# lschoe/mpyc

Hardware: AMD Instinct MI355X
Metric: field-ops/sec (modmul + share+recombine) on 10^7-elt SecFld array (higher is better)
Workload: dtype u64; 1 GPU; configs[1]: SecFld(GF(2^61-1)) array, 10^7 elements per GPU; step = modmul + np_random_split(m=3,t=1, coefficients supplied) + np_recombine(k=3); modmul is fused into the share-generation kernel (product never written to HBM); n_per_gpu=10000000, prime=2^61-1, m=3, t=1, k=3, buffer_sets=4, parallelism=element-sharded x1, no collective

## Files before the change

### mpyc_amd/csrc/api.hip

```cpp
#include <hip/hip_runtime.h>
#include <stdint.h>
#include <stdio.h>
#include <stdlib.h>
#include <string.h>
#include <limits.h>
#include <mutex>
#include <new>

#include "../../include/ffgpu.h"
#include "../../include/ffgpu_math.h"
#include "handoff.hpp"
#include "kernels.hpp"
#include "policy_build.hpp"

using namespace ffgpu;

const FieldOps* ffgpu_ops_pm64_mersenne();
const FieldOps* ffgpu_ops_pm64_k64();
const FieldOps* ffgpu_ops_pm64_gen();
const FieldOps* ffgpu_ops_rc64();
const FieldOps* ffgpu_ops_rc32();
const FieldOps* ffgpu_ops_pm128_k128();
const FieldOps* ffgpu_ops_pm128_gen();
const FieldOps* ffgpu_ops_pm96();
// ... 137 lines not shown

static void acc_harvest(ffgpu_ctx* c) {
    if (c->acc_n == 0) return;
    (void)hipEventSynchronize(c->acc_ev[2 * (c->acc_n - 1) + 1]);
    for (int i = 0; i < c->acc_n; ++i) {
        float ms = 0.f;
        if (hipEventElapsedTime(&ms, c->acc_ev[2 * i], c->acc_ev[2 * i + 1]) == hipSuccess) c->acc_ms += ms;
    }
    c->acc_calls += (unsigned long long)c->acc_n;
    c->acc_n = 0;
}

struct LaunchTimer {
    ffgpu_ctx* c;
    hipStream_t st;
    int slot;
    LaunchTimer(ffgpu_ctx* ctx, hipStream_t s) : c(ctx && ctx->timing ? ctx : nullptr), st(s), slot(-1) {
        if (!c) return;
        if (c->timing == 2) {
            if (c->acc_n == ffgpu_ctx::ACC_MAX) acc_harvest(c);
            if (c->acc_n == c->acc_made) {
                if (hipEventCreate(&c->acc_ev[2 * c->acc_made]) != hipSuccess ||
                    hipEventCreate(&c->acc_ev[2 * c->acc_made + 1]) != hipSuccess) {
                    c = nullptr;
                    return;
                }
                ++c->acc_made;
            }
            slot = c->acc_n++;
            (void)hipEventRecord(c->acc_ev[2 * slot], st);
        } else {
            (void)hipEventRecord(c->ev0, st);
        }
    }
    ~LaunchTimer() {
        if (!c) return;
        if (slot >= 0) {
            (void)hipEventRecord(c->acc_ev[2 * slot + 1], st);
        } else {
            (void)hipEventRecord(c->ev1, st);
            c->timed = 1;
        }
    }
};

struct CallScope {
    DeviceGuard dev;
    LaunchTimer timer;
    hipStream_t st;
    LaunchCfg lc;
    CallScope(ffgpu_ctx* ctx, void* stream)
        : dev(ctx->device), timer(ctx, (hipStream_t)stream), st((hipStream_t)stream), lc(ctx->lc) {}
    CallScope(ffgpu_ctx* ctx, void* stream, int kind, const ByteRange* in, int nin, const ByteRange& out) : CallScope(ctx, stream) {
        if (lc.handoff) {
            std::lock_guard<std::mutex> lk(ctx->handoff_mu);
            int fed = 0;
            const int keep = ctx->handoff.launch(stream, kind, in, nin, &out, 1, &fed);
            lc.policy = (keep ? (kind == HK_SPLIT ? CP_ST_SC1 : CP_ST_PLAIN) : CP_ST_NT) | (fed ? CP_FED : 0);
        }
    }
};

static const FieldOps* ops_for(int kind) {
    switch (kind) {
        case POL_PM64_MERSENNE: return ffgpu_ops_pm64_mersenne();
        case POL_PM64_K64: return ffgpu_ops_pm64_k64();
        case POL_PM64_GEN: return ffgpu_ops_pm64_gen();
        case POL_RC64: return ffgpu_ops_rc64();
        case POL_RC32: return ffgpu_ops_rc32();
        case POL_PM128_K128: return ffgpu_ops_pm128_k128();
        case POL_PM128_GEN: return ffgpu_ops_pm128_gen();
        case POL_PM96: return ffgpu_ops_pm96();
        case POL_PM192: return ffgpu_ops_pm192();
        case POL_MONT192: return ffgpu_ops_mont192();
        case POL_MONT128: return ffgpu_ops_mont128();
        case POL_GF2P8: return ffgpu_ops_gf2p8();
        case POL_GF2W32: return ffgpu_ops_gf2w32();
        case POL_GF2W64: return ffgpu_ops_gf2w64();
        case POL_GF2W128: return ffgpu_ops_gf2w128();
        default: return nullptr;
    }
}

extern "C" {

int ffgpu_abi_version(void) { return FFGPU_ABI_VERSION; }

const char* ffgpu_strerror(int status) {
    switch (status) {
        case FFGPU_OK: return "ok";
        case FFGPU_EINVAL: return "invalid argument";
        case FFGPU_ENOTSUP: return "field or size not supported by this build";
        case FFGPU_EHIP: return "HIP runtime error";
        case FFGPU_ESTALE: return "interprocess mapping does not show the exported row (stale mapping)";
        case FFGPU_EMODULUS: return "unusable modulus";
        case FFGPU_ENOMEM: return "out of device memory";
        default: return "unknown status";
    }
}

const char* ffgpu_last_hip_error(void) { return g_hip_err; }

int ffgpu_device_count(int* count) {
    if (!count) return FFGPU_EINVAL;
    int n = 0;
    hipError_t e = hipGetDeviceCount(&n);
    if (e != hipSuccess) {
        *count = 0;
        return hip_fail(e, "hipGetDeviceCount");
    }
    *count = n;
    return FFGPU_OK;
}

int ffgpu_device_pci_bus_id(int device, char* buf, int len) {
    if (!buf || len < 16 || device < 0) return FFGPU_EINVAL;
    buf[0] = 0;
    hipError_t e = hipDeviceGetPCIBusId(buf, len, device);
    if (e != hipSuccess) return hip_fail(e, "hipDeviceGetPCIBusId");
    return FFGPU_OK;
}

struct Switch {
    const char* name;
    int LaunchCfg::*field;
    double LaunchCfg::*real;
    double def;
    int lowest, highest;
};
static const Switch SWITCHES[] = {
    {"FFGPU_BLOCKS_PER_CU", &LaunchCfg::blocks_per_cu, nullptr, 0, 0, INT_MAX},
    {"FFGPU_MM_MFMA", &LaunchCfg::mm_mfma, nullptr, 1, INT_MIN, INT_MAX},
    {"FFGPU_MM_MFMA_MIN", nullptr, &LaunchCfg::mm_mfma_min, 8e7, 0, 0},
    {"FFGPU_MM_STACK_LOOP_MIN", &LaunchCfg::mm_stack_loop_min, nullptr, 1 << 22, 0, INT_MAX},
    {"FFGPU_GF2W_BITSLICED", &LaunchCfg::gf2w_bitsliced, nullptr, 1, INT_MIN, INT_MAX},
    {"FFGPU_HANDOFF", &LaunchCfg::handoff, nullptr, 1, INT_MIN, INT_MAX},
    {"FFGPU_CONV_WIDE_PER_CU", &LaunchCfg::conv_wide_per_cu, nullptr, 2, 0, INT_MAX},
    {"FFGPU_SCAN_GEOM", &LaunchCfg::scan_geom, nullptr, 0, 0, 2},
    {"FFGPU_SCAN_TILE_THREADS", &LaunchCfg::scan_tile_threads, nullptr, 256, 1, 256},
};

int ffgpu_ctx_create(int kind, const uint64_t* modulus, int nlimbs, int device, ffgpu_ctx** out) {
    if (!modulus || !out || nlimbs < 1 || nlimbs > 3 || device < 0) return FFGPU_EINVAL;
    PolicyBlob pb;
    memset(&pb, 0, sizeof(pb));
    int rc;
    if (kind == FFGPU_PRIME) {
        rc = build_prime_policy3(&pb, modulus, nlimbs);
    } else if (kind == FFGPU_BINARY) {
        rc = build_binary_policy(&pb, modulus, nlimbs);
    } else {
        rc = FFGPU_EINVAL;
    }
    if (rc != FFGPU_OK) return rc;
    if (!ops_for(pb.kind)) return FFGPU_ENOTSUP;
    ffgpu_ctx* c = new (std::nothrow) ffgpu_ctx();
    if (!c) return FFGPU_ENOMEM;
    c->ops = ops_for(pb.kind);
    c->kind = kind;
    c->device = device;
    for (int i = 0; i < nlimbs; ++i) c->modulus[i] = modulus[i];
    memcpy(c->policy, pb.bytes, sizeof(c->policy));
    c->reduction = pb.reduction;
    c->elem_bytes = pb.elem_bytes;
    c->policy_kind = pb.kind;
    rng_const(pb, c->rng_r);
    {
        int cus = 256;
        if (hipDeviceGetAttribute(&cus, hipDeviceAttributeMultiprocessorCount, device) != hipSuccess || cus <= 0) cus = 256;
        c->lc.num_cu = cus;
        for (const Switch& sw : SWITCHES) {
            const char* e = getenv(sw.name);
            if (sw.real) {
                c->lc.*sw.real = e ? atof(e) : sw.def;
                continue;
            }
            const int v = e ? atoi(e) : (int)sw.def;
            c->lc.*sw.field = v >= sw.lowest && v <= sw.highest ? v : (int)sw.def;
        }
    }
    if (pb.kind == POL_GF2W64 || pb.kind == POL_GF2W128) {
        bool in_regs;
        if (pb.kind == POL_GF2W128) {
            GF2W128 f;
            memcpy(&f, pb.bytes, sizeof(f));
            in_regs = (f.fast & 1) != 0;
        } else {
            GF2W64 f;
            memcpy(&f, pb.bytes, sizeof(f));
// ... 430 lines not shown
                void* dev_singular, void* stream) {
    ARGCHK(ctx && n >= 0 && ncols >= n && (mode == 0 || mode == 1));
    if (batch == 0) return FFGPU_OK;
    ARGCHK(dev_singular && (mode == 0 || det_out));
    if (n == 0) return FFGPU_OK;
    ARGCHK(a);
    CallScope cs(ctx, stream);
    ExpArgs ex;
    inverse_exponent(ctx, &ex);
    HIPCHK(hipMemsetAsync(dev_singular, 0, batch * sizeof(int), cs.st));
    return status_of(ctx->ops->gauss(ctx->policy, cs.lc, a, n, ncols, batch, mode, &ex,
                                     mode ? det_out : nullptr, (int*)dev_singular, cs.st));
}

int ffgpu_inv(ffgpu_ctx* ctx, const void* a, void* out, size_t n, void* dev_zero_flag, void* stream) {
    ARGCHK(ctx);
    if (n == 0) return FFGPU_OK;
    ARGCHK(a && out);
    ExpArgs ex;
    inverse_exponent(ctx, &ex);
    CallScope cs(ctx, stream);
    return status_of(ctx->ops->inv(ctx->policy, cs.lc, a, &ex, out, n, (int*)dev_zero_flag, cs.st));
}

int ffgpu_beaver_combine(ffgpu_ctx* ctx, const void* z, const void* x, const void* y, const void* d, const void* e,
                         int add_de, void* out, size_t n, void* stream) {
    ARGCHK(ctx);
    if (n == 0) return FFGPU_OK;
    ARGCHK(z && x && y && d && e && out);
    CallScope cs(ctx, stream);
    return status_of(ctx->ops->beaver(ctx->policy, cs.lc, z, x, y, d, e, out, add_de ? 1 : 0, n,
                                      cs.st));
}

static int split_inputs(const ffgpu_ctx* ctx, const void* a, const void* b, const void* coeffs, int t, size_t coeff_stride, size_t n,
                        ByteRange in[3]) {
    int nin = 0;
    in[nin++] = byte_range(a, rows_bytes(ctx, 1, 0, n));
    if (b) in[nin++] = byte_range(b, rows_bytes(ctx, 1, 0, n));
    if (coeffs) in[nin++] = byte_range(coeffs, rows_bytes(ctx, (size_t)t, coeff_stride, n));
    return nin;
}

static int do_split(ffgpu_ctx* ctx, const void* a, const void* b, bool fused, const void* coeffs,
                    size_t coeff_stride, int t, int m, void* shares, size_t share_stride, size_t n,
                    void* stream) {
    ARGCHK(ctx);
    ARGCHK(m >= 1 && t >= 0 && t < m);
    if (n == 0) return FFGPU_OK;
    ARGCHK(a && shares && (!fused || b) && (t == 0 || coeffs));
    ARGCHK((m == 1 || share_stride >= n) && (t <= 1 || coeff_stride >= n));
    ByteRange in[3];
    const int nin = split_inputs(ctx, a, fused ? b : nullptr, t > 0 ? coeffs : nullptr, t, coeff_stride, n, in);
    CallScope cs(ctx, stream, HK_SPLIT, in, nin, byte_range(shares, rows_bytes(ctx, (size_t)m, share_stride, n)));
    return status_of(ctx->ops->split(ctx->policy, cs.lc, a, fused ? b : nullptr, coeffs,
                                     coeff_stride, t, m, shares, share_stride, n, cs.st,
                                     nullptr));
}

static int make_rng(const ffgpu_ctx* ctx, const uint8_t* key32, uint64_t nonce, int rounds, RngArgs* ra) {
    if (!key32) return FFGPU_EINVAL;
    if (rounds == 0) rounds = 20;
    if (rounds != 20 && rounds != 12 && rounds != 8) return FFGPU_EINVAL;
    memset(ra, 0, sizeof(*ra));
    memcpy(ra->rk.key, key32, 32);
    ra->rk.nonce[0] = (uint32_t)nonce;
    ra->rk.nonce[1] = (uint32_t)(nonce >> 32);
    ra->rk.rounds = (uint32_t)rounds;
    ra->r0 = ctx->rng_r[0];
    ra->r1 = ctx->rng_r[1];
    return FFGPU_OK;
}

static RngArgs make_dev_rng(const ffgpu_ctx* ctx, void* dev_state, uint64_t nonce_off, int defer_advance, bool sampler) {
    RngArgs ra;
    memset(&ra, 0, sizeof(ra));
    ra.rk.rounds = 20;
    if (sampler) {
        ra.r0 = ctx->rng_r[0];
        ra.r1 = ctx->rng_r[1];
    }
    ra.dev_key = (const RngKey*)dev_state;
    ra.nonce_off = (uint32_t)nonce_off;
    ra.no_advance = defer_advance ? 1 : 0;
    return ra;
}

static int do_split_rng(ffgpu_ctx* ctx, const void* a, const void* b, bool fused, const uint8_t* key32,
                        uint64_t nonce, int rounds, int t, int m, void* shares, size_t share_stride, size_t n,
                        void* stream) {
    ARGCHK(ctx);
    ARGCHK(m >= 1 && t >= 0 && t < m);
    RngArgs ra;
    int rc = make_rng(ctx, key32, nonce, rounds, &ra);
    if (rc != FFGPU_OK) return rc;
    if (n == 0) return FFGPU_OK;
    ARGCHK(a && shares && (!fused || b));
    ARGCHK(m == 1 || share_stride >= n);
    ByteRange in[3];
    const int nin = split_inputs(ctx, a, fused ? b : nullptr, nullptr, 0, 0, n, in);
    CallScope cs(ctx, stream, HK_SPLIT, in, nin, byte_range(shares, rows_bytes(ctx, (size_t)m, share_stride, n)));
    if (fused && t > 0) ra.aux = gf8_tables_on_device(ctx);
    return status_of(ctx->ops->split(ctx->policy, cs.lc, a, fused ? b : nullptr, nullptr, 0, t, m,
                                     shares, share_stride, n, cs.st, t > 0 ? &ra : nullptr));
}
int ffgpu_ctx_scalar_limbs(const ffgpu_ctx* ctx) { return (ctx && ctx->elem_bytes == 24) ? 3 : 2; }

size_t ffgpu_rng_state_bytes(void) { return sizeof(RngKey); }

int ffgpu_rng_state_init(ffgpu_ctx* ctx, void* dev_state, const uint8_t* host_key32, uint64_t nonce, int rounds,
                         void* stream) {
    ARGCHK(ctx && dev_state);
    RngArgs ra;
    int rc = make_rng(ctx, host_key32, nonce, rounds, &ra);
    if (rc != FFGPU_OK) return rc;
    CallScope cs(ctx, stream);
    HIPCHK(hipMemcpyAsync(dev_state, &ra.rk, sizeof(RngKey), hipMemcpyHostToDevice, cs.st));
    HIPCHK(hipStreamSynchronize(cs.st));
    return FFGPU_OK;
}

int ffgpu_split_rng_state(ffgpu_ctx* ctx, const void* secrets, const void* mul_by, void* dev_state, int t, int m,
                          void* shares, size_t share_stride, size_t n, void* stream) {
    ARGCHK(ctx && dev_state);
    ARGCHK(m >= 1 && t >= 0 && t < m);
    if (n == 0) return FFGPU_OK;
    ARGCHK(secrets && shares && (m == 1 || share_stride >= n));
    RngArgs ra = make_dev_rng(ctx, dev_state, 0, 0, true);
    ByteRange in[3];
    const int nin = split_inputs(ctx, secrets, mul_by, nullptr, 0, 0, n, in);
    CallScope cs(ctx, stream, HK_SPLIT, in, nin, byte_range(shares, rows_bytes(ctx, (size_t)m, share_stride, n)));
    if (mul_by && t > 0) ra.aux = gf8_tables_on_device(ctx);
    return status_of(ctx->ops->split(ctx->policy, cs.lc, secrets, mul_by, nullptr, 0, t, m, shares, share_stride, n, cs.st,
                                     t > 0 ? &ra : nullptr));
}

int ffgpu_gate_rng(ffgpu_ctx* ctx, const void* const* host_rows_a, const uint64_t* host_lambda_a, int ka,
                   const void* const* host_rows_b, const uint64_t* host_lambda_b, int kb, const uint8_t* host_key32,
                   uint64_t nonce, int rounds, void* dev_state, int t, int m, void* shares, size_t share_stride,
                   size_t n, void* stream) {
    return ffgpu_gate_rng_batch(ctx, host_rows_a, host_lambda_a, ka, 0, host_rows_b, host_lambda_b, kb, 0, host_key32,
                                dev_state ? 0 : nonce, rounds, dev_state, 0, t, m, shares, share_stride, 0, n, 1, stream);
}

int ffgpu_rng_state_advance(ffgpu_ctx* ctx, void* dev_state, uint32_t by, void* stream) {
    ARGCHK(ctx && dev_state);
    if (by == 0) return FFGPU_OK;
    DeviceGuard g(ctx->device);
    hipLaunchKernelGGL((k_rng_advance<0>), dim3(1), dim3(1), 0, (hipStream_t)stream, (RngKey*)dev_state, by);
    return status_of(launched());
}

int ffgpu_gate_rng_batch(ffgpu_ctx* ctx, const void* const* host_rows_a, const uint64_t* host_lambda_a, int ka,
                         size_t batch_stride_a, const void* const* host_rows_b, const uint64_t* host_lambda_b, int kb,
                         size_t batch_stride_b, const uint8_t* host_key32, uint64_t nonce, int rounds, void* dev_state,
                         int defer_advance, int t, int m, void* shares, size_t share_stride, size_t batch_stride_out,
                         size_t n, int nbatch, void* stream) {
    ARGCHK(ctx);
    ARGCHK(nbatch >= 1 && nbatch <= 255);
    ARGCHK(!dev_state || nonce <= 0xffffffffull);
    ARGCHK(dev_state || nbatch == 1 || nonce < (1ull << 40));
    ARGCHK(m >= 1 && t >= 1 && t < m && ka >= 1 && kb >= 0);
    if (t > 3 || ka > 7 || kb > 7) return FFGPU_ENOTSUP;
    ARGCHK(host_rows_a && host_lambda_a && (kb == 0 || (host_rows_b && host_lambda_b)));
    RngArgs ra;
    if (dev_state) {
        ra = make_dev_rng(ctx, dev_state, nonce, defer_advance, true);
    } else {
        int rc = make_rng(ctx, host_key32, nonce, rounds, &ra);
        if (rc != FFGPU_OK) return rc;
    }
    if (n == 0) return FFGPU_OK;
    ARGCHK(shares && (m == 1 || share_stride >= n));
    for (int j = 0; j < ka; ++j) ARGCHK(host_rows_a[j]);
    for (int j = 0; j < kb; ++j) ARGCHK(host_rows_b[j]);
    ByteRange in[14];
    int nin = 0;
    for (int j = 0; j < ka; ++j) in[nin++] = byte_range(host_rows_a[j], rows_bytes(ctx, (size_t)nbatch, batch_stride_a, n));
    for (int j = 0; j < kb; ++j) in[nin++] = byte_range(host_rows_b[j], rows_bytes(ctx, (size_t)nbatch, batch_stride_b, n));
    const size_t oelems = ((size_t)nbatch - 1) * batch_stride_out + ((size_t)m - 1) * share_stride + n;
    CallScope cs(ctx, stream, HK_SPLIT, in, nin, byte_range(shares, oelems * (size_t)ctx->elem_bytes));
    ra.aux = gf8_tables_on_device(ctx);
    return status_of(ctx->ops->gate(ctx->policy, cs.lc, host_rows_a, host_lambda_a, ka, host_rows_b,
                                    host_lambda_b, kb, t, m, shares, share_stride, n, cs.st, &ra,
// ... 1112 lines not shown
```

### mpyc_amd/csrc/handoff.hpp

```cpp
#pragma once
#include <stddef.h>
#include <stdint.h>

namespace ffgpu {

struct ByteRange {
    uintptr_t lo, hi;
};
inline ByteRange byte_range(const void* p, size_t bytes) {
    const uintptr_t lo = (uintptr_t)p;
    return {lo, lo + bytes};
}
inline bool overlaps(const ByteRange& a, const ByteRange& b) { return a.lo < b.hi && b.lo < a.hi && a.lo < a.hi && b.lo < b.hi; }

enum HandoffKind { HK_EW = 0, HK_SPLIT = 1, HK_REC = 2, HK_COPY = 3, HK_KINDS = 4 };

struct HandoffTracker {
    enum { STREAMS = 8, ROWS = 8 };
    static constexpr size_t MAX_KEEP_BYTES = (size_t)256 << 20;
    struct Lane {
        const void* stream;
        uint64_t stamp;
        int used;
        int kind;
        int nout;
        int kept;
        ByteRange out[ROWS];
        uint8_t keep[HK_KINDS];
    } lanes[STREAMS];
    uint64_t clock;

    void reset() {
        for (Lane& l : lanes) {
            l.stream = nullptr;
            l.stamp = 0;
            l.used = 0;
            l.kind = 0;
            l.nout = 0;
            l.kept = 0;
            for (uint8_t& k : l.keep) k = 0;
        }
        clock = 0;
    }
    Lane& lane_of(const void* stream) {
        Lane* victim = nullptr;
        for (Lane& l : lanes) {
            if (l.used && l.stream == stream) return l;
            if (!victim || (!l.used && victim->used) || (l.used == victim->used && l.stamp < victim->stamp)) victim = &l;
        }
        Lane& l = *victim;
        l.stream = stream;
        l.used = 1;
        l.nout = 0;
        l.kept = 0;
        for (uint8_t& k : l.keep) k = 0;
        return l;
    }
    int launch(const void* stream, int kind, const ByteRange* in, int nin, const ByteRange* out, int nout, int* fed_in = nullptr) {
        Lane& l = lane_of(stream);
        l.stamp = ++clock;
        bool fed = false;
        if (l.nout > 0) {
            for (int i = 0; i < nin && !fed; ++i)
                for (int j = 0; j < l.nout && !fed; ++j) fed = overlaps(in[i], l.out[j]);
            l.keep[l.kind] = fed ? 1 : 0;
        }
        if (fed_in) *fed_in = fed && l.kept;
        size_t bytes = 0;
        for (int j = 0; j < nout; ++j) bytes += out[j].hi > out[j].lo ? out[j].hi - out[j].lo : 0;
        const int keep = l.keep[kind] && bytes <= MAX_KEEP_BYTES;
        l.kind = kind;
        l.kept = keep;
        l.nout = nout < ROWS ? nout : ROWS;
        for (int j = 0; j < l.nout; ++j) l.out[j] = out[j];
        return keep;
    }
};

}
```

### mpyc_amd/csrc/kernels.hpp

```cpp
#pragma once
#include <hip/hip_runtime.h>
#include <stdint.h>
#include <stdlib.h>
#include <string.h>
#include <type_traits>
#include <utility>
#include "fields.hpp"
#include "rng.hpp"

namespace ffgpu {

enum { BLOCK = 256 };
enum EwOp { OP_ADD = 0, OP_SUB = 1, OP_MUL = 2, OP_RSUB = 3, OP_NEG = 4, OP_REDUCE = 5 };

enum { MAXK = 9, MAXW = 8, MAXK_ANY = 64, MAXT = 4 };

template <class W>
struct alignas(16) Pack {
    enum { N = 16 / sizeof(W) };
    W w[N];
};
template <>
struct Pack<u192e> {
    enum { N = 1 };
// ... 132 lines not shown
__device__ __forceinline__ X24Raw ldgw_issue(const u192e* p) {
    const ff_u32x4* base = x24_wave_base(p);
    const uint32_t lane = __lane_id();
    X24Raw r;
    if constexpr (NT) {
        r.r0 = __builtin_nontemporal_load(base + lane);
        r.r1 = __builtin_nontemporal_load(base + 64 + (lane & 31));
    } else {
        r.r0 = base[lane];
        r.r1 = base[64 + (lane & 31)];
    }
    return r;
}
__device__ __forceinline__ Pack<u192e> ldgw_finish(const X24Raw& raw) {
    const uint32_t lane = __lane_id();
    x24_lds4* L = x24_region();
    X24_LDS_FENCE();
    L[lane] = raw.r0;
    L[64 + (lane & 31)] = raw.r1;
    X24_LDS_FENCE();
    const x24_lds2* R = reinterpret_cast<const x24_lds2*>(L) + 3 * lane;
    const ff_u32x2 a0 = R[0], a1 = R[1], b = R[2];
    Pack<u192e> r;
    r.w[0].lo = (uint64_t)a0.x | ((uint64_t)a0.y << 32);
    r.w[0].mid = (uint64_t)a1.x | ((uint64_t)a1.y << 32);
    r.w[0].hi = (uint64_t)b.x | ((uint64_t)b.y << 32);
    return r;
}
template <bool NT>
__device__ __forceinline__ void stgw(u192e* p, const Pack<u192e>& x) {
    ff_u32x4* base = x24_wave_base(p);
    const uint32_t lane = __lane_id();
    x24_lds4* L = x24_region();
    x24_lds2* R = reinterpret_cast<x24_lds2*>(L) + 3 * lane;
    ff_u32x2 a0, a1, b;
    a0.x = (uint32_t)x.w[0].lo;  a0.y = (uint32_t)(x.w[0].lo >> 32);
    a1.x = (uint32_t)x.w[0].mid; a1.y = (uint32_t)(x.w[0].mid >> 32);
    b.x = (uint32_t)x.w[0].hi;   b.y = (uint32_t)(x.w[0].hi >> 32);
    X24_LDS_FENCE();
    R[0] = a0;
    R[1] = a1;
    R[2] = b;
    X24_LDS_FENCE();
    const ff_u32x4 r0 = L[lane], r1 = L[64 + (lane & 31)];
    if constexpr (NT) {
        __builtin_nontemporal_store(r0, base + lane);
        __builtin_nontemporal_store(r1, base + 64 + (lane & 31));
    } else {
        base[lane] = r0;
        base[64 + (lane & 31)] = r1;
    }
}

enum CachePolicy { CP_ST_NT = 0, CP_ST_PLAIN = 1, CP_ST_SC1 = 2, CP_ST_MASK = 3, CP_FED = 4 };
#define FF_STORE_FENCE(p) asm volatile("" ::"v"(p) : "memory")
template <class P>
__device__ __forceinline__ void stg_sc1(P* p, const P& x) {
    static_assert(sizeof(P) == 16, "16-byte packs only");
    ff_u32x4 v;
    __builtin_memcpy(&v, &x, 16);
    asm volatile("global_store_dwordx4 %0, %1, off sc1\n\ts_nop 1" ::"v"(p), "v"(v) : "memory");
}
template <class P, class X>
__device__ __forceinline__ void stg_plain(P* p, const X& x) {
    FF_STORE_FENCE(p);
    stg<false>(p, x);
    FF_STORE_FENCE(p);
}
template <bool NT, class P, class X>
__device__ __forceinline__ void stg_k(P* p, const X& x, int pol) {
    const int st = pol & CP_ST_MASK;
    if constexpr (std::is_same<P, X>::value && sizeof(P) == 16) {
        if (st == CP_ST_SC1) {
            stg_sc1(p, x);
            return;
        }
    }
    if (st != CP_ST_NT) stg_plain(p, x);
    else stg<NT>(p, x);
}
template <bool NT, class P, class X>
__device__ __forceinline__ void stgw_k(P* p, const X& x, int pol) {
    if constexpr (std::is_same<P, u192e>::value) {
        if ((pol & CP_ST_MASK) != CP_ST_NT) {
            FF_STORE_FENCE(p);
            stgw<false>(p, x);
            FF_STORE_FENCE(p);
        } else {
            stgw<NT>(p, x);
        }
    } else {
        stg_k<NT>(p, x, pol);
    }
}

template <class F>
__device__ __forceinline__ typename F::word ld_elem(const typename F::elem* p, size_t i) {
    if constexpr (sizeof(typename F::elem) == 12) {
        typename F::word w;
        w.lo = (uint64_t)p[i].x[0] | ((uint64_t)p[i].x[1] << 32);
        w.hi = p[i].x[2];
        return w;
    } else if constexpr (F::EPW == 1) {
        return p[i];
    } else {
        return (typename F::word)p[i];
    }
}
template <class F>
__device__ __forceinline__ void st_elem(typename F::elem* p, size_t i, typename F::word w) {
    if constexpr (sizeof(typename F::elem) == 12) {
        p[i].x[0] = (uint32_t)w.lo;
        p[i].x[1] = (uint32_t)(w.lo >> 32);
        p[i].x[2] = (uint32_t)w.hi;
    } else if constexpr (F::EPW == 1) {
        p[i] = w;
    } else {
        p[i] = (typename F::elem)w;
    }
}

template <int N, class At>
__device__ __forceinline__ auto reg_select(int idx, At at) {
    auto v = at(0);
#pragma unroll
    for (int x = 1; x < N; ++x) {
        const auto a = at(x);
        v = (x == idx) ? a : v;
    }
    return v;
}
template <class F, int N>
__device__ __forceinline__ typename F::word drawn_elem(const typename F::word (&pack)[N], size_t e) {
    typedef typename F::word W;
    W v = reg_select<N>((int)((e % (N * F::EPW)) / F::EPW), [&](int q) { return pack[q]; });
    if constexpr (F::EPW > 1) v = (W)((v >> (8 * (e % F::EPW))) & 0xffu);
    return v;
}

template <class F, int OP>
__device__ __forceinline__ typename F::word ew_apply(const F& f, typename F::word a, typename F::word b) {
    if constexpr (OP == OP_ADD) return f.add(a, b);
    else if constexpr (OP == OP_SUB) return f.sub(a, b);
    else if constexpr (OP == OP_MUL) return f.mul(a, b);
    else if constexpr (OP == OP_RSUB) return f.sub(b, a);
    else if constexpr (OP == OP_NEG) return f.neg(a);
// ... 178 lines not shown
#pragma unroll
                for (int q = 0; q < P::N; ++q) acc[q].mac(f, lam[j0 + u], x[u].w[q]);
            }
    }
    P r;
#pragma unroll
    for (int q = 0; q < P::N; ++q) r.w[q] = acc[q].reduce(f);
    return r;
}
template <class F>
__device__ __forceinline__ typename F::word gate_load_elem(const F& f, const typename F::elem* const* rows,
                                                           const typename F::word* lam, int k, size_t e) {
    typename F::acc acc;
    f.acc_zero(acc);
    for (int j = 0; j < k; ++j) {
        f.acc_mac(acc, lam[j], ld_elem<F>(rows[j], e));
    }
    return f.acc_reduce(acc);
}

__device__ __forceinline__ void rng_state_release(const RngArgs& ra) {
    if (!ra.dev_key || !ra.release) return;
    __syncthreads();
    if (threadIdx.x == 0) {
        RngKey* st = const_cast<RngKey*>(ra.dev_key);
        __threadfence();
        const uint32_t done = atomicAdd(&st->pad_, 1u);
        if (done == gridDim.x * gridDim.y - 1) {
            st->pad_ = 0;
            if (++st->nonce[0] == 0) st->nonce[1] += 65536u;
            __threadfence();
        }
    }
}

template <int UNUSED>
__global__ void k_rng_advance(RngKey* st, uint32_t by) {
    if (threadIdx.x == 0 && blockIdx.x == 0) {
        const uint32_t old = st->nonce[0];
        st->nonce[0] = old + by;
        if (st->nonce[0] < old) st->nonce[1] += 65536u;
    }
}
__device__ __forceinline__ void rng_load_state(RngArgs& ra) {
    if (ra.dev_key) {
        ra.rk = *ra.dev_key;
        const uint32_t old = ra.rk.nonce[0];
        ra.rk.nonce[0] = old + ra.nonce_off;
        if (ra.rk.nonce[0] < old) ra.rk.nonce[1] += 65536u;
    }
}
enum { RNG_RELEASE_MAX_GRID = 512 };

template <class F, int T, bool FUSE_MUL, bool NT, bool RNG, bool REC = false>
__global__ __launch_bounds__(BLOCK) void k_split(F f, const typename F::elem* __restrict__ a,
                                                  const typename F::elem* __restrict__ b,
                                                  const typename F::elem* __restrict__ coef, size_t cstride,
                                                  int m, typename F::elem* __restrict__ out, size_t ostride,
                                                  size_t nvec, size_t n, RngArgs ra, GateSrc<F> gs, int pol) {
    rng_load_state(ra);
    size_t yoffA = 0, yoffB = 0;
    if constexpr (REC) {
        const size_t yb = blockIdx.y;
        yoffA = yb * gs.yA;
        yoffB = yb * gs.yB;
        out += yb * gs.yO;
        ra.rk.nonce[1] += (uint32_t)yb << 8;
    }
    typedef Pack<typename F::word> P;
    typedef typename MemPack<F>::type MP;
    typedef typename F::word W;
    constexpr int TT = T > 0 ? T : 1;
    constexpr bool WC = !RNG && !REC;
    const size_t gid = (size_t)blockIdx.x * BLOCK + threadIdx.x;
    const size_t gsz = (size_t)gridDim.x * BLOCK;
    const MP* __restrict__ av = reinterpret_cast<const MP*>(a);
    const MP* __restrict__ bv = reinterpret_cast<const MP*>(b);
    constexpr int G = (RNG && T > 0) ? RngLayout<F, TT, P::N>::G : 1;
    constexpr int EPV_ = P::N * F::EPW;
    const size_t npacks_all = (n + EPV_ - 1) / EPV_;
    const size_t ngroups = (RNG && T > 0) ? (npacks_all + G - 1) / G : nvec;
    constexpr bool TABMUL = (F::EPW == 4) && FUSE_MUL && RNG;
    __shared__ uint16_t s_lg[TABMUL ? 256 : 1];
    __shared__ uint32_t s_ex[TABMUL ? 256 : 1];
    if constexpr (TABMUL) {
        if (ra.aux) {
            s_lg[threadIdx.x] = reinterpret_cast<const uint16_t*>(ra.aux)[threadIdx.x];
            s_ex[threadIdx.x] = reinterpret_cast<const uint32_t*>(reinterpret_cast<const char*>(ra.aux) + 512)[threadIdx.x];
            __syncthreads();
        }
    }
    decltype(ldgw_issue<NT>(av)) rc[TT];
    auto load_s = [&](size_t i) -> P {
        P s, s2;
        if constexpr (REC) {
            const size_t iA = i + yoffA / EPV_, iB = i + yoffB / EPV_;
            s = gs.plainA ? ldg<NT>(reinterpret_cast<const MP*>(gs.rowsA[0]) + iA)
                          : gate_load<F, NT>(f, gs.rowsA, gs.lamA, gs.kA, iA);
            s2 = gs.square ? s
                           : (gs.plainB ? ldg<NT>(reinterpret_cast<const MP*>(gs.rowsB[0]) + iB)
                                        : gate_load<F, NT>(f, gs.rowsB, gs.lamB, gs.kB, iB));
        } else {
            if constexpr (WC) {
                const auto rs = ldgw_issue<NT>(av + i);
                auto rs2 = rs;
                if constexpr (FUSE_MUL) rs2 = ldgw_issue<NT>(bv + i);
#pragma unroll
                for (int j = 0; j < T; ++j) rc[j] = ldgw_issue<NT>(reinterpret_cast<const MP*>(coef + (size_t)j * cstride) + i);
                s = ldgw_finish(rs);
                if constexpr (FUSE_MUL) s2 = ldgw_finish(rs2);
            } else {
                s = ldg<NT>(av + i);
                if constexpr (FUSE_MUL) s2 = ldg<NT>(bv + i);
            }
        }
        if constexpr (TABMUL) {
            if (ra.aux) {
                const uint8_t* ex = reinterpret_cast<const uint8_t*>(s_ex);
#pragma unroll
                for (int q = 0; q < P::N; ++q) {
                    uint32_t acc = 0;
#pragma unroll
                    for (int k8 = 0; k8 < 4; ++k8) {
                        const uint32_t lsum = (uint32_t)s_lg[((uint32_t)s.w[q] >> (8 * k8)) & 0xffu] +
                                              (uint32_t)s_lg[((uint32_t)s2.w[q] >> (8 * k8)) & 0xffu];
                        acc |= (uint32_t)ex[lsum] << (8 * k8);
                    }
                    s.w[q] = (W)acc;
                }
            } else {
#pragma unroll
                for (int q = 0; q < P::N; ++q) s.w[q] = f.mul(s.w[q], s2.w[q]);
            }
        } else if constexpr (FUSE_MUL) {
#pragma unroll
            for (int q = 0; q < P::N; ++q) s.w[q] = f.mul(s.w[q], s2.w[q]);
        }
        return s;
    };
    auto eval_store = [&](size_t i, const P& s, W (&c)[TT][P::N]) {
        if constexpr (!(RNG && T > 0)) {
            if constexpr (WC) {
#pragma unroll
                for (int j = 0; j < T; ++j) {
                    const P t_ = ldgw_finish(rc[j]);
#pragma unroll
                    for (int q = 0; q < P::N; ++q) c[j][q] = t_.w[q];
                }
            } else {
#pragma unroll
                for (int j = 0; j < T; ++j) {
                    const P t_ = ldg<NT>(reinterpret_cast<const MP*>(coef + (size_t)j * cstride) + i);
#pragma unroll
                    for (int q = 0; q < P::N; ++q) c[j][q] = t_.w[q];
                }
            }
        }
        if constexpr (!F::BINARY && T >= 1) {
            W dd[P::N][TT];
#pragma unroll
            for (int q = 0; q < P::N; ++q) {
                W cq[TT];
#pragma unroll
                for (int j = 0; j < T; ++j) cq[j] = c[j][q];
                share_diff_init<F, TT>(f, cq, dd[q]);
            }
            P y = s;
            for (int party = 1; party <= m; ++party) {
#pragma unroll
                for (int q = 0; q < P::N; ++q) y.w[q] = share_diff_next<F, TT>(f, y.w[q], dd[q]);
                if constexpr (WC) stgw_k<NT>(reinterpret_cast<MP*>(out + (size_t)(party - 1) * ostride) + i, y, pol);
                else stg_k<NT>(reinterpret_cast<MP*>(out + (size_t)(party - 1) * ostride) + i, y, pol);
            }
        } else {
            for (int party = 1; party <= m; ++party) {
                P y;
                if constexpr (T == 0) {
                    y = s;
                } else {
#pragma unroll
                    for (int q = 0; q < P::N; ++q) {
                        W acc = c[T - 1][q];
#pragma unroll
                        for (int j = T - 2; j >= 0; --j) acc = f.muladd_small(acc, (uint32_t)party, c[j][q]);
                        y.w[q] = f.muladd_small(acc, (uint32_t)party, s.w[q]);
                    }
                }
                if constexpr (WC) stgw_k<NT>(reinterpret_cast<MP*>(out + (size_t)(party - 1) * ostride) + i, y, pol);
                else stg_k<NT>(reinterpret_cast<MP*>(out + (size_t)(party - 1) * ostride) + i, y, pol);
            }
        }
    };
    if (RNG && T > 0 && G > 1 && ra.spread) {
        for (size_t i = gid; i < nvec; i += gsz) {
            W c[TT][P::N];
            const P s = load_s(i);
            rng_draw_pack<F, TT, P::N>(f, ra.rk, ra.r0, ra.r1, (uint64_t)i, (uint64_t)npacks_all, c);
            eval_store(i, s, c);
        }
    } else {
        for (size_t ig = gid; ig < ngroups; ig += gsz) {
            W cg[G][TT][P::N];
            P sv[G];
            if constexpr (REC) {
                rng_draw_group<F, TT, P::N>(f, ra.rk, ra.r0, ra.r1, (uint64_t)ig, cg);
#pragma unroll
                for (int u = 0; u < G; ++u) {
                    const size_t i = (size_t)u * ngroups + ig;
                    if (i < nvec) {
                        sv[0] = load_s(i);
                        eval_store(i, sv[0], cg[u]);
                    }
                }
                continue;
            }
#pragma unroll
            for (int u = 0; u < G; ++u) {
                const size_t i = (size_t)u * ngroups + ig;
                if (i < nvec) sv[u] = load_s(i);
            }
            if constexpr (RNG && T > 0) rng_draw_group<F, TT, P::N>(f, ra.rk, ra.r0, ra.r1, (uint64_t)ig, cg);
#pragma unroll
            for (int u = 0; u < G; ++u) {
                const size_t i = (size_t)u * ngroups + ig;
                if (i < nvec) eval_store(i, sv[u], cg[u]);
            }
        }
    }
    constexpr int EPV = P::N * F::EPW;
    const size_t done = nvec * (size_t)EPV;
    for (size_t e = done + gid; e < n; e += gsz) {
        W s;
        if constexpr (REC) {
            const size_t eA = e + yoffA, eB = e + yoffB;
            s = gs.plainA ? ld_elem<F>(gs.rowsA[0], eA) : gate_load_elem<F>(f, gs.rowsA, gs.lamA, gs.kA, eA);
            s = f.mul(s, gs.square ? s
                                   : (gs.plainB ? ld_elem<F>(gs.rowsB[0], eB)
                                                : gate_load_elem<F>(f, gs.rowsB, gs.lamB, gs.kB, eB)));
        } else {
            s = ld_elem<F>(a, e);
            if constexpr (FUSE_MUL) s = f.mul(s, ld_elem<F>(b, e));
        }
// ... 1290 lines not shown
```

### mpyc_amd/csrc/launch.hpp

```cpp
#pragma once

namespace ffgpu {

struct LaunchCfg {
    int num_cu;
    int blocks_per_cu;
    int mm_mfma;
    double mm_mfma_min;
    int gf2w_bitsliced;
    int conv_wide_per_cu;
    int scan_geom;
    int scan_tile_threads;
    int mm_stack_loop_min;
    int handoff;
    int policy;
};

enum LaunchCode {
    L_OK = 0,
    L_BAD_ARG,
    L_NOT_SUPPORTED,
    L_DECLINED,
    L_PLAN_REFUSED,
    L_WS_TOO_SMALL,
    L_HIP_ERROR
};
struct LaunchStatus {
    LaunchCode code;
    hipError_t hip;
    LaunchStatus(LaunchCode c = L_OK, hipError_t e = hipSuccess) : code(c), hip(e) {}
    bool ok() const { return code == L_OK; }
};
inline LaunchStatus launched() {
    const hipError_t e = hipGetLastError();
    return e == hipSuccess ? LaunchStatus() : LaunchStatus(L_HIP_ERROR, e);
}
#define FFGPU_CHECK_LAUNCH()                      \
    do {                                          \
        const LaunchStatus s__ = launched();      \
        if (!s__.ok()) return s__;                \
    } while (0)

inline unsigned grid_for(size_t iters, const LaunchCfg& lc) {
    size_t want = (iters + BLOCK - 1) / BLOCK;
    size_t cap = lc.blocks_per_cu > 0 ? (size_t)lc.blocks_per_cu * (size_t)lc.num_cu : (size_t)0x7fffffff;
    if (want < 1) want = 1;
    return (unsigned)(want < cap ? want : cap);
}

inline bool aligned16(const void* p) { return ((uintptr_t)p & 15u) == 0; }

struct FieldOps {
    LaunchStatus (*ew2)(const void* F, const LaunchCfg& lc, int op, const void* a, const void* b, void* o, size_t n,
               hipStream_t st);
    LaunchStatus (*ew1)(const void* F, const LaunchCfg& lc, int op, const void* a, const uint64_t* scalar2, void* o,
               size_t n, hipStream_t st);
    LaunchStatus (*muladd)(const void* F, const LaunchCfg& lc, const void* a, const void* b, const void* c, void* o,
                  size_t n, hipStream_t st);
    LaunchStatus (*split)(const void* F, const LaunchCfg& lc, const void* a, const void* b, const void* coef,
                 size_t cstride, int t, int m, void* out, size_t ostride, size_t n, hipStream_t st,
                 const RngArgs* rng);
    LaunchStatus (*rng_coeffs)(const void* F, const LaunchCfg& lc, void* coef, size_t cstride, int t, size_t n, hipStream_t st,
                      const RngArgs* rng);
    LaunchStatus (*recombine)(const void* F, const LaunchCfg& lc, const void* const* rows, const uint64_t* lam2, int k,
                     int w, void* out, size_t ostride, size_t n, hipStream_t st);
    LaunchStatus (*pow)(const void* F, const LaunchCfg& lc, const void* a, const ExpArgs* ex, void* out, size_t n, hipStream_t st);
    LaunchStatus (*inv)(const void* F, const LaunchCfg& lc, const void* a, const ExpArgs* ex, void* out, size_t n, int* flag,
// ... 193 lines not shown
        }
    }
    static const F& policy(const void* Fp) { return *reinterpret_cast<const F*>(Fp); }
    static bool stride_ok(size_t stride) { return (stride * sizeof(E)) % PACK_ALIGN == 0; }

    template <int OP>
    static void go_ew2(const F& f, const LaunchCfg& lc, const E* a, const E* b, E* o, size_t n, hipStream_t st) {
        const Plan p = plan(n, al(a) && al(b) && al(o), lc);
        constexpr int OCC = EwOccupancy<F, OP>::waves;
        if constexpr (OCC > 0)
            hipLaunchKernelGGL((k_ew2_occ<F, OP, true, OCC>), dim3(p.grid), dim3(BLOCK), 0, st, f, a, b, o, p.nvec, n, p.pol);
        else
            hipLaunchKernelGGL((k_ew2<F, OP, true>), dim3(p.grid), dim3(BLOCK), 0, st, f, a, b, o, p.nvec, n, p.pol);
    }
    static LaunchStatus ew2(const void* Fp, const LaunchCfg& lc, int op, const void* a, const void* b, void* o, size_t n,
                   hipStream_t st) {
        const F& f = policy(Fp);
        const E* A = (const E*)a;
        const E* B = (const E*)b;
        E* O = (E*)o;
        const bool known = dispatch_int(std::integer_sequence<int, OP_ADD, OP_SUB, OP_MUL>(), op,
                                        [&](auto o_) { go_ew2<decltype(o_)::value>(f, lc, A, B, O, n, st); });
        return known ? launched() : LaunchStatus(L_BAD_ARG);
    }

    template <int OP>
    static void go_ew1(const F& f, const LaunchCfg& lc, const E* a, W s, E* o, size_t n, hipStream_t st) {
        const Plan p = plan(n, al(a) && al(o), lc);
        hipLaunchKernelGGL((k_ew1<F, OP, true>), dim3(p.grid), dim3(BLOCK), 0, st, f, a, s, o, p.nvec, n, p.pol);
    }
    static LaunchStatus ew1(const void* Fp, const LaunchCfg& lc, int op, const void* a, const uint64_t* scalar2, void* o,
                   size_t n, hipStream_t st) {
        const F& f = policy(Fp);
        W s = scalar2 ? word_at<F>(f, scalar2, 0) : word_from_limbs<F>(f, 0, 0);
        const E* A = (const E*)a;
        E* O = (E*)o;
        const bool known = dispatch_int(std::integer_sequence<int, OP_ADD, OP_RSUB, OP_MUL, OP_NEG, OP_REDUCE>(), op,
                                        [&](auto o_) { go_ew1<decltype(o_)::value>(f, lc, A, s, O, n, st); });
        return known ? launched() : LaunchStatus(L_BAD_ARG);
    }

    static LaunchStatus muladd(const void* Fp, const LaunchCfg& lc, const void* a, const void* b, const void* c, void* o,
                      size_t n, hipStream_t st) {
        const F& f = policy(Fp);
        const Plan p = plan(n, al(a) && al(b) && al(c) && al(o), lc);
        hipLaunchKernelGGL((k_muladd<F, true>), dim3(p.grid), dim3(BLOCK), 0, st, f, (const E*)a,
                           (const E*)b, (const E*)c, (E*)o, p.nvec, n, p.pol);
        return launched();
    }

    template <int T, bool FUSE, bool RNG, bool REC = false>
    static void go_split(const F& f, const Plan& p, const E* a, const E* b, const E* coef, size_t cstride, int m, E* out,
                         size_t ostride, size_t n, hipStream_t st, const RngArgs& ra, const GateSrc<F>& gs, unsigned gy = 1) {
        hipLaunchKernelGGL((k_split<F, T, FUSE, true, RNG, REC>), dim3(p.grid, gy), dim3(BLOCK), 0, st, f, a, b,
                           coef, cstride, m, out, ostride, p.nvec, n, ra, gs, p.pol);
    }
    template <bool FUSE, bool RNG>
    static LaunchStatus split_t(const F& f, const LaunchCfg& lc, const E* a, const E* b, const E* coef, size_t cstride,
                       int t, int m, E* out, size_t ostride, size_t n, hipStream_t st, const RngArgs& ra_in) {
        RngArgs ra = ra_in;
        if (t > MAXT) {
            const Plan p = RNG ? plan_rng(n, false, lc, ra) : plan(n, false, lc);
            hipLaunchKernelGGL((k_split_any<F, FUSE, RNG>), dim3(p.grid), dim3(BLOCK), 0, st, f, a, b, coef, cstride,
                               t, m, out, ostride, n, ra);
        } else {
            const bool vec = al(a) && (!FUSE || al(b)) && al(out) &&
                             (stride_ok(ostride) || m <= 1) &&
                             (RNG || t == 0 || (al(coef) && (stride_ok(cstride) || t <= 1)));
            const Plan p = RNG ? plan_rng(n, vec, lc, ra) : plan(n, vec, lc);
            GateSrc<F> gs;
            memset(&gs, 0, sizeof(gs));
            const bool known = dispatch_int(IntRange<0, MAXT>(), t, [&](auto t_) {
                constexpr int T = decltype(t_)::value;
                go_split<T, FUSE, (T > 0 && RNG)>(f, p, a, b, coef, cstride, m, out, ostride, n, st, ra, gs);
            });
            if (!known) return L_BAD_ARG;
        }
        if (RNG && t > 0) rng_advance(ra, st);
        return L_OK;
    }
    static LaunchStatus gate(const void* Fp, const LaunchCfg& lc, const void* const* rowsA, const uint64_t* lamA2, int kA,
                    const void* const* rowsB, const uint64_t* lamB2, int kB, int t, int m, void* out, size_t ostride,
                    size_t n, hipStream_t st, const RngArgs* rng, int nbatch, size_t yA, size_t yB, size_t yO) {
        const F& f = policy(Fp);
        if (t < 1 || t > 3 || kA < 1 || kA > GATE_MAXK || kB < 0 || kB > GATE_MAXK || !rng) return L_NOT_SUPPORTED;
        if (nbatch < 1 || nbatch > 255) return L_NOT_SUPPORTED;
        GateSrc<F> gs;
        memset(&gs, 0, sizeof(gs));
        bool vec = al(out) && (stride_ok(ostride) || m <= 1);
        if (nbatch > 1) {
            gs.yA = yA;
            gs.yB = yB;
            gs.yO = yO;
            vec = vec && stride_ok(yA) && stride_ok(yO) && (kB == 0 || stride_ok(yB));
        }
        for (int j = 0; j < kA; ++j) {
            gs.rowsA[j] = (const E*)rowsA[j];
            gs.lamA[j] = f.prep(word_at<F>(f, lamA2, j));
            vec = vec && al(rowsA[j]);
        }
        for (int j = 0; j < kB; ++j) {
            gs.rowsB[j] = (const E*)rowsB[j];
            gs.lamB[j] = f.prep(word_at<F>(f, lamB2, j));
            vec = vec && al(rowsB[j]);
        }
        gs.kA = kA;
        gs.kB = kB;
        gs.square = kB == 0;
// ... 1267 lines not shown
```

Before: 256.4 billion field-ops/s.

## Track cache-retention decisions per share row in split handoff

The handoff tracker now records which individual share rows of a split output are read by the next launch. When the whole output exceeds a byte budget (about 240 MB by default), only the rows that were actually consumed, up to that budget, are stored with the cache-retaining policy, and the rest use non-temporal stores. This goes through a per-row policy bitmask and a new kernel template variant. The aim is to keep the data recombine reads resident in the MI355X's large last-level cache instead of dropping all retention once the output is too large. The cost is extra host bookkeeping and another kernel instantiation, and the budget may not match the real cache capacity.

```diff
diff --git a/mpyc_amd/csrc/api.hip b/mpyc_amd/csrc/api.hip
--- a/mpyc_amd/csrc/api.hip
+++ b/mpyc_amd/csrc/api.hip
@@ -213,13 +213,32 @@
     CallScope(ffgpu_ctx* ctx, void* stream)
         : dev(ctx->device), timer(ctx, (hipStream_t)stream), st((hipStream_t)stream), lc(ctx->lc) {}
     CallScope(ffgpu_ctx* ctx, void* stream, int kind, const ByteRange* in, int nin, const ByteRange& out) : CallScope(ctx, stream) {
-        if (lc.handoff) {
+        if (lc.handoff) track(ctx, kind, in, nin, out);
+    }
+    CallScope(ffgpu_ctx* ctx, void* stream, const ByteRange* in, int nin, const void* shares, int m, size_t stride, size_t n)
+        : CallScope(ctx, stream) {
+        const size_t eb = (size_t)ctx->elem_bytes;
+        if (lc.handoff && lc.handoff_keep_kb < 0) {
+            track(ctx, HK_SPLIT, in, nin, byte_range(shares, ((size_t)(m - 1) * stride + n) * eb));
+        } else if (lc.handoff) {
+            ByteRange rows[HandoffTracker::ROWS + 1];
+            const int ROWS = HandoffTracker::ROWS, nrows = m <= ROWS ? m : ROWS + 1;
+            for (int j = 0; j < nrows; ++j) rows[j] = byte_range((const char*)shares + (size_t)j * stride * eb, n * eb);
+            if (m > ROWS) rows[ROWS].hi = rows[ROWS].lo + ((size_t)(m - ROWS - 1) * stride + n) * eb;
             std::lock_guard<std::mutex> lk(ctx->handoff_mu);
             int fed = 0;
-            const int keep = ctx->handoff.launch(stream, kind, in, nin, &out, 1, &fed);
-            lc.policy = (keep ? (kind == HK_SPLIT ? CP_ST_SC1 : CP_ST_PLAIN) : CP_ST_NT) | (fed ? CP_FED : 0);
+            const unsigned keep =
+                ctx->handoff.launch_rows(st, HK_SPLIT, in, nin, rows, nrows, (size_t)lc.handoff_keep_kb << 10, &fed);
+            lc.policy = (keep ? CP_ST_SC1 | rows_field(keep) : CP_ST_NT) | (fed ? CP_FED : 0);
         }
     }
+    void track(ffgpu_ctx* ctx, int kind, const ByteRange* in, int nin, const ByteRange& out) {
+        std::lock_guard<std::mutex> lk(ctx->handoff_mu);
+        int fed = 0;
+        const int keep = ctx->handoff.launch(st, kind, in, nin, &out, 1, &fed);
+        lc.policy = (keep ? (kind == HK_SPLIT ? CP_ST_SC1 | rows_field(~0u) : CP_ST_PLAIN) : CP_ST_NT) | (fed ? CP_FED : 0);
+    }
+    static int rows_field(unsigned mask) { return (int)((mask & ((1u << CP_ROWS) - 1)) << CP_ROWS_SHIFT); }
 };
 
 static const FieldOps* ops_for(int kind) {
@@ -289,6 +308,7 @@
     double def;
     int lowest, highest;
 };
+enum { HANDOFF_KEEP_KB = 240000000 / 1024 };
 static const Switch SWITCHES[] = {
     {"FFGPU_BLOCKS_PER_CU", &LaunchCfg::blocks_per_cu, nullptr, 0, 0, INT_MAX},
     {"FFGPU_MM_MFMA", &LaunchCfg::mm_mfma, nullptr, 1, INT_MIN, INT_MAX},
@@ -296,6 +316,7 @@
     {"FFGPU_MM_STACK_LOOP_MIN", &LaunchCfg::mm_stack_loop_min, nullptr, 1 << 22, 0, INT_MAX},
     {"FFGPU_GF2W_BITSLICED", &LaunchCfg::gf2w_bitsliced, nullptr, 1, INT_MIN, INT_MAX},
     {"FFGPU_HANDOFF", &LaunchCfg::handoff, nullptr, 1, INT_MIN, INT_MAX},
+    {"FFGPU_HANDOFF_KEEP_KB", &LaunchCfg::handoff_keep_kb, nullptr, HANDOFF_KEEP_KB, -1, 256 << 10},
     {"FFGPU_CONV_WIDE_PER_CU", &LaunchCfg::conv_wide_per_cu, nullptr, 2, 0, INT_MAX},
     {"FFGPU_SCAN_GEOM", &LaunchCfg::scan_geom, nullptr, 0, 0, 2},
     {"FFGPU_SCAN_TILE_THREADS", &LaunchCfg::scan_tile_threads, nullptr, 256, 1, 256},
@@ -832,7 +853,7 @@
     ARGCHK((m == 1 || share_stride >= n) && (t <= 1 || coeff_stride >= n));
     ByteRange in[3];
     const int nin = split_inputs(ctx, a, fused ? b : nullptr, t > 0 ? coeffs : nullptr, t, coeff_stride, n, in);
-    CallScope cs(ctx, stream, HK_SPLIT, in, nin, byte_range(shares, rows_bytes(ctx, (size_t)m, share_stride, n)));
+    CallScope cs(ctx, stream, in, nin, shares, m, share_stride, n);
     return status_of(ctx->ops->split(ctx->policy, cs.lc, a, fused ? b : nullptr, coeffs,
                                      coeff_stride, t, m, shares, share_stride, n, cs.st,
                                      nullptr));
@@ -879,7 +900,7 @@
     ARGCHK(m == 1 || share_stride >= n);
     ByteRange in[3];
     const int nin = split_inputs(ctx, a, fused ? b : nullptr, nullptr, 0, 0, n, in);
-    CallScope cs(ctx, stream, HK_SPLIT, in, nin, byte_range(shares, rows_bytes(ctx, (size_t)m, share_stride, n)));
+    CallScope cs(ctx, stream, in, nin, shares, m, share_stride, n);
     if (fused && t > 0) ra.aux = gf8_tables_on_device(ctx);
     return status_of(ctx->ops->split(ctx->policy, cs.lc, a, fused ? b : nullptr, nullptr, 0, t, m,
                                      shares, share_stride, n, cs.st, t > 0 ? &ra : nullptr));
@@ -909,7 +930,7 @@
     RngArgs ra = make_dev_rng(ctx, dev_state, 0, 0, true);
     ByteRange in[3];
     const int nin = split_inputs(ctx, secrets, mul_by, nullptr, 0, 0, n, in);
-    CallScope cs(ctx, stream, HK_SPLIT, in, nin, byte_range(shares, rows_bytes(ctx, (size_t)m, share_stride, n)));
+    CallScope cs(ctx, stream, in, nin, shares, m, share_stride, n);
     if (mul_by && t > 0) ra.aux = gf8_tables_on_device(ctx);
     return status_of(ctx->ops->split(ctx->policy, cs.lc, secrets, mul_by, nullptr, 0, t, m, shares, share_stride, n, cs.st,
                                      t > 0 ? &ra : nullptr));
diff --git a/mpyc_amd/csrc/handoff.hpp b/mpyc_amd/csrc/handoff.hpp
--- a/mpyc_amd/csrc/handoff.hpp
+++ b/mpyc_amd/csrc/handoff.hpp
@@ -27,6 +27,8 @@
         int kept;
         ByteRange out[ROWS];
         uint8_t keep[HK_KINDS];
+        uint8_t kept_rows;
+        uint8_t read_rows[HK_KINDS];
     } lanes[STREAMS];
     uint64_t clock;
 
@@ -35,12 +37,17 @@
             l.stream = nullptr;
             l.stamp = 0;
             l.used = 0;
-            l.kind = 0;
-            l.nout = 0;
-            l.kept = 0;
-            for (uint8_t& k : l.keep) k = 0;
+            forget(l);
         }
         clock = 0;
+    }
+    static void forget(Lane& l) {
+        l.kind = 0;
+        l.nout = 0;
+        l.kept = 0;
+        l.kept_rows = 0;
+        for (uint8_t& k : l.keep) k = 0;
+        for (uint8_t& r : l.read_rows) r = 0;
     }
     Lane& lane_of(const void* stream) {
         Lane* victim = nullptr;
@@ -51,29 +58,65 @@
         Lane& l = *victim;
         l.stream = stream;
         l.used = 1;
-        l.nout = 0;
-        l.kept = 0;
-        for (uint8_t& k : l.keep) k = 0;
+        forget(l);
         return l;
     }
+    static unsigned settle(Lane& l, const ByteRange* in, int nin) {
+        unsigned read = 0;
+        for (int j = 0; j < l.nout; ++j)
+            for (int i = 0; i < nin; ++i)
+                if (overlaps(in[i], l.out[j])) {
+                    read |= 1u << j;
+                    break;
+                }
+        if (l.nout > 0) {
+            l.keep[l.kind] = read ? 1 : 0;
+            l.read_rows[l.kind] = (uint8_t)read;
+        }
+        return read;
+    }
+    void remember(Lane& l, int kind, const ByteRange* out, int nout, unsigned kept_rows) {
+        l.kind = kind;
+        l.kept = kept_rows ? 1 : 0;
+        l.kept_rows = (uint8_t)kept_rows;
+        l.nout = nout < ROWS ? nout : ROWS;
+        for (int j = 0; j < l.nout; ++j) l.out[j] = out[j];
+    }
+    static size_t bytes_of(const ByteRange& r) { return r.hi > r.lo ? r.hi - r.lo : 0; }
     int launch(const void* stream, int kind, const ByteRange* in, int nin, const ByteRange* out, int nout, int* fed_in = nullptr) {
         Lane& l = lane_of(stream);
         l.stamp = ++clock;
-        bool fed = false;
-        if (l.nout > 0) {
-            for (int i = 0; i < nin && !fed; ++i)
-                for (int j = 0; j < l.nout && !fed; ++j) fed = overlaps(in[i], l.out[j]);
-            l.keep[l.kind] = fed ? 1 : 0;
+        const unsigned read = settle(l, in, nin);
+        if (fed_in) *fed_in = (read & l.kept_rows) != 0;
+        size_t bytes = 0;
+        for (int j = 0; j < nout; ++j) bytes += bytes_of(out[j]);
+        const int keep = l.keep[kind] && bytes <= MAX_KEEP_BYTES;
+        remember(l, kind, out, nout, keep ? (1u << ROWS) - 1 : 0);
+        return keep;
+    }
+    unsigned launch_rows(const void* stream, int kind, const ByteRange* in, int nin, const ByteRange* rows, int nrows,
+                         size_t budget_bytes, int* fed_in = nullptr) {
+        Lane& l = lane_of(stream);
+        l.stamp = ++clock;
+        const unsigned read = settle(l, in, nin);
+        if (fed_in) *fed_in = (read & l.kept_rows) != 0;
+        const int nr = nrows < ROWS ? nrows : ROWS;
+        size_t bytes = 0;
+        for (int j = 0; j < nrows; ++j) bytes += bytes_of(rows[j]);
+        unsigned mask = 0;
+        if (bytes <= budget_bytes) {
+            if (l.keep[kind]) mask = (1u << nr) - 1;
+        } else {
+            size_t used = 0;
+            for (int j = 0; j < nr; ++j) {
+                if (!(l.read_rows[kind] >> j & 1)) continue;
+                if (bytes_of(rows[j]) > budget_bytes - used) break;
+                used += bytes_of(rows[j]);
+                mask |= 1u << j;
+            }
         }
-        if (fed_in) *fed_in = fed && l.kept;
-        size_t bytes = 0;
-        for (int j = 0; j < nout; ++j) bytes += out[j].hi > out[j].lo ? out[j].hi - out[j].lo : 0;
-        const int keep = l.keep[kind] && bytes <= MAX_KEEP_BYTES;
-        l.kind = kind;
-        l.kept = keep;
-        l.nout = nout < ROWS ? nout : ROWS;
-        for (int j = 0; j < l.nout; ++j) l.out[j] = out[j];
-        return keep;
+        remember(l, kind, rows, nrows, mask);
+        return mask;
     }
 };
 
diff --git a/mpyc_amd/csrc/kernels.hpp b/mpyc_amd/csrc/kernels.hpp
--- a/mpyc_amd/csrc/kernels.hpp
+++ b/mpyc_amd/csrc/kernels.hpp
@@ -208,7 +208,7 @@
     }
 }
 
-enum CachePolicy { CP_ST_NT = 0, CP_ST_PLAIN = 1, CP_ST_SC1 = 2, CP_ST_MASK = 3, CP_FED = 4 };
+enum CachePolicy { CP_ST_NT = 0, CP_ST_PLAIN = 1, CP_ST_SC1 = 2, CP_ST_MASK = 3, CP_FED = 4, CP_ROWS_SHIFT = 3, CP_ROWS = 8 };
 #define FF_STORE_FENCE(p) asm volatile("" ::"v"(p) : "memory")
 template <class P>
 __device__ __forceinline__ void stg_sc1(P* p, const P& x) {
@@ -248,6 +248,16 @@
     } else {
         stg_k<NT>(p, x, pol);
     }
+}
+
+__device__ __forceinline__ int row_pol(int pol, int j) {
+    return (j < CP_ROWS && ((pol >> (CP_ROWS_SHIFT + j)) & 1)) ? pol : (pol & ~CP_ST_MASK);
+}
+
+inline bool rows_differ(int pol, int m) {
+    if ((pol & CP_ST_MASK) == CP_ST_NT) return false;
+    const int want = (1 << (m < CP_ROWS ? m : CP_ROWS)) - 1;
+    return m > CP_ROWS || ((pol >> CP_ROWS_SHIFT) & want) != want;
 }
 
 template <class F>
@@ -532,7 +542,7 @@
 }
 enum { RNG_RELEASE_MAX_GRID = 512 };
 
-template <class F, int T, bool FUSE_MUL, bool NT, bool RNG, bool REC = false>
+template <class F, int T, bool FUSE_MUL, bool NT, bool RNG, bool REC = false, bool ROWS = false>
 __global__ __launch_bounds__(BLOCK) void k_split(F f, const typename F::elem* __restrict__ a,
                                                   const typename F::elem* __restrict__ b,
                                                   const typename F::elem* __restrict__ coef, size_t cstride,
@@ -618,6 +628,10 @@
         }
         return s;
     };
+    auto pol_of = [&](int j) {
+        if constexpr (ROWS) return row_pol(pol, j);
+        else return pol;
+    };
     auto eval_store = [&](size_t i, const P& s, W (&c)[TT][P::N]) {
         if constexpr (!(RNG && T > 0)) {
             if constexpr (WC) {
@@ -649,8 +663,8 @@
             for (int party = 1; party <= m; ++party) {
 #pragma unroll
                 for (int q = 0; q < P::N; ++q) y.w[q] = share_diff_next<F, TT>(f, y.w[q], dd[q]);
-                if constexpr (WC) stgw_k<NT>(reinterpret_cast<MP*>(out + (size_t)(party - 1) * ostride) + i, y, pol);
-                else stg_k<NT>(reinterpret_cast<MP*>(out + (size_t)(party - 1) * ostride) + i, y, pol);
+                if constexpr (WC) stgw_k<NT>(reinterpret_cast<MP*>(out + (size_t)(party - 1) * ostride) + i, y, pol_of(party - 1));
+                else stg_k<NT>(reinterpret_cast<MP*>(out + (size_t)(party - 1) * ostride) + i, y, pol_of(party - 1));
             }
         } else {
             for (int party = 1; party <= m; ++party) {
@@ -666,8 +680,8 @@
                         y.w[q] = f.muladd_small(acc, (uint32_t)party, s.w[q]);
                     }
                 }
-                if constexpr (WC) stgw_k<NT>(reinterpret_cast<MP*>(out + (size_t)(party - 1) * ostride) + i, y, pol);
-                else stg_k<NT>(reinterpret_cast<MP*>(out + (size_t)(party - 1) * ostride) + i, y, pol);
+                if constexpr (WC) stgw_k<NT>(reinterpret_cast<MP*>(out + (size_t)(party - 1) * ostride) + i, y, pol_of(party - 1));
+                else stg_k<NT>(reinterpret_cast<MP*>(out + (size_t)(party - 1) * ostride) + i, y, pol_of(party - 1));
             }
         }
     };
diff --git a/mpyc_amd/csrc/launch.hpp b/mpyc_amd/csrc/launch.hpp
--- a/mpyc_amd/csrc/launch.hpp
+++ b/mpyc_amd/csrc/launch.hpp
@@ -13,6 +13,7 @@
     int scan_tile_threads;
     int mm_stack_loop_min;
     int handoff;
+    int handoff_keep_kb;
     int policy;
 };
 
@@ -312,8 +313,12 @@
     template <int T, bool FUSE, bool RNG, bool REC = false>
     static void go_split(const F& f, const Plan& p, const E* a, const E* b, const E* coef, size_t cstride, int m, E* out,
                          size_t ostride, size_t n, hipStream_t st, const RngArgs& ra, const GateSrc<F>& gs, unsigned gy = 1) {
-        hipLaunchKernelGGL((k_split<F, T, FUSE, true, RNG, REC>), dim3(p.grid, gy), dim3(BLOCK), 0, st, f, a, b,
-                           coef, cstride, m, out, ostride, p.nvec, n, ra, gs, p.pol);
+        if (rows_differ(p.pol, m))
+            hipLaunchKernelGGL((k_split<F, T, FUSE, true, RNG, REC, true>), dim3(p.grid, gy), dim3(BLOCK), 0, st, f, a, b,
+                               coef, cstride, m, out, ostride, p.nvec, n, ra, gs, p.pol);
+        else
+            hipLaunchKernelGGL((k_split<F, T, FUSE, true, RNG, REC>), dim3(p.grid, gy), dim3(BLOCK), 0, st, f, a, b,
+                               coef, cstride, m, out, ostride, p.nvec, n, ra, gs, p.pol);
     }
     template <bool FUSE, bool RNG>
     static LaunchStatus split_t(const F& f, const LaunchCfg& lc, const E* a, const E* b, const E* coef, size_t cstride,
```

Result: no change. 255.8 billion field-ops/s (-0.2%).
